# tum-pbs/differentiable-piso

Hardware: AMD Instinct MI355X
Metric: PISO steps/s (fwd+adjoint) at 2048^2 staggered grid (higher is better)
Workload: dtype f64

## Files before the change

### differentiable-piso_amd/csrc/cg.hip

```cpp
#include <atomic>
#include "cg_kernels.h"
#include "cg_driver.h"
#include "cg_tiny.h"
#include "options.h"
#include <cstdio>
#include <vector>

namespace piso {

struct CgProfile {
  int enabled = 0, stride = 8;
  double ms[4] = {0, 0, 0, 0};
  long long count[4] = {0, 0, 0, 0};
};
static CgProfile g_prof;

struct HostPoll {
  CgState* pinned = nullptr;
  hipEvent_t ev[2] = {nullptr, nullptr};
  hipEvent_t seg_ev[2] = {nullptr, nullptr};
  int cus = 0;
};
static std::atomic<unsigned> g_persist_launches{0};
static int g_persist_fallbacks = 0;
static thread_local int tl_xcd_map[kPersistMaxGrid];
static thread_local int tl_xcd_map_n = 0;
static long long g_tiny_solves = 0;
enum { DI_PATH = 0, DI_SIZEOF_T, DI_SIZEOF_CT, DI_V, DI_RECON, DI_SYMMETRIC, DI_ROWS_PER_WAVE, DI_K1_GRID, DI_K1_TILES, DI_R, DI_NQ,
       DI_WAVES, DI_LAUNCH_GRID, DI_PADDED, DI_XCD_LOCAL, DI_FELL_BACK, DI_TINY_PER_X, DI_K2_GRID, DI_SEGMENTS, DI_COUNT };
static thread_local int tl_dispatch[DI_COUNT];
static thread_local int tl_dispatch_n = 0;
static bool g_xcd_local_failed = false;
static long long g_verify_runs = 0;
static int g_verify_failures = 0;
constexpr int kPollDevices = 16;
static thread_local HostPoll tl_poll_dev[kPollDevices];
static thread_local HostPoll* tl_poll_cur = &tl_poll_dev[0];
#define tl_poll (*tl_poll_cur)

static int ensure_poll() {
  int dev = 0;
// ... 180 lines not shown

  int start(unsigned* persist_ws, bool symmetric, int rank_deficient, bool allow_persist) {
    const size_t n = (size_t)a.nx * a.ny;
    tile = cg_tile(a, V, opt(OPT_CG_RPW), opt(OPT_CG_MAXBLOCKS));
    PISO_TRY(ensure_poll());
    if (prof) PISO_TRY(ensure_events(ep));
    ep.used[0] = ep.used[1] = 0;
    prof_stride = g_prof.stride > 0 ? g_prof.stride : 8;
    cg_init<T><<<tile.gflat, kBlock, 0, stream>>>(a, rank_deficient);
    PISO_LAUNCH_CHECK();
    batch = poll_batch(n);
    plan = persist_plan(PersistQuery{a.nx, a.ny, V, a.per_y, a.nx_true != 0, sizeof(T), sizeof(CT), RECON, symmetric, false, tl_poll.cus,
                                     opt(OPT_CG_PERSIST), opt(OPT_CG_PERSIST_R), opt(OPT_CG_PERSIST_HALF), opt(OPT_CG_PERSIST_NQ),
                                     opt(OPT_CG_XCD_LOCAL), g_xcd_local_failed, allow_persist});
    PISO_TRY((persist_prepare<T, CT, RECON, false>(plan, tl_poll.cus, pc, persist_ws, stream)));
    if (plan.R && kPersistDiag && opt_on(OPT_CG_PERSIST_TIMING)) {
      PISO_HIP_CHECK(hipMalloc(reinterpret_cast<void**>(&timing.ticks), 12 * plan.launch_grid * sizeof(unsigned long long)));
      PISO_HIP_CHECK(hipMemsetAsync(timing.ticks, 0, 12 * plan.launch_grid * sizeof(unsigned long long), stream));
      pc.timing = timing.ticks;
    }
    record_dispatch(plan.R ? 3 : 2, sizeof(T), sizeof(CT), 0, V, RECON, symmetric, &tile, &plan, !allow_persist);
    seg_len = persist_segment_len(n, opt(OPT_CG_SEGMENT));
    hipEvent_t* seg_ev = tl_poll.seg_ev;
    if (plan.R && prof && !seg_ev[0]) { PISO_HIP_CHECK(hipEventCreate(&seg_ev[0])); PISO_HIP_CHECK(hipEventCreate(&seg_ev[1])); }
    return PISO_OK;
  }

  bool persistent() const { return plan.R != 0; }
  int segment(int k, int ke, CgLoop& st) {
    hipEvent_t* seg_ev = tl_poll.seg_ev;
// ... 51 lines not shown
    return PISO_OK;
  }
  int look(int k, CgLoop& st) { return (!fixed && (k + 1) % batch == 0 && k + 1 < st.total) ? poll(st, false) : PISO_OK; }

  int finish(CgLoop& st) {
    if (!fixed && !st.finished) PISO_TRY(poll(st, true));
    PISO_HIP_CHECK(hipStreamSynchronize(stream));
    if (opt(OPT_CG_XCD_MAP) == 1) {
      tl_xcd_map_n = 0;
      if (st.segments_run > 0 && !plan.xcd_local && plan.grid <= kPersistMaxGrid) {
        PISO_HIP_CHECK(hipMemcpy(tl_xcd_map, pc.xcd + kPersistXcdTable, (size_t)plan.grid * sizeof(int), hipMemcpyDeviceToHost));
        tl_xcd_map_n = plan.grid;
      }
    }
    if (st.segments_run > 0) {
      int herr = 0;
      PISO_HIP_CHECK(hipMemcpy(&herr, pc.err, sizeof(int), hipMemcpyDeviceToHost));
      if (herr) { ++g_persist_fallbacks; return kPersistRetry; }
    }
    if (st.segments_run > 0 && sizeof(T) == 8 && !fixed && opt(OPT_CG_VERIFY) != 0) {
      bool failed = false;
      PISO_TRY((verify_residual<T, CT>(a, pc, stream, &failed)));
      if (failed) { ++g_verify_failures; ++g_persist_fallbacks; return kPersistRetry; }
    }
    if (timing.ticks) PISO_TRY(print_persist_timing(timing.ticks, plan.grid, st.k_last));
    tl_dispatch[DI_SEGMENTS] = st.segments_run;
    return PISO_OK;
  }
};

template <typename T>
__global__ __launch_bounds__(kBlock) void cg_copy_rows(const T* __restrict__ src, T* __restrict__ dst, int nx, int ny, int ld_src, int ld_dst) {
  const size_t n = (size_t)nx * ny;
// ... 165 lines not shown
                          1 << 30, iterations, nullptr, kernel_ms_out, workspace, workspace_bytes, stream);
}

void piso_cg_profile_enable(int enable, int stride) {
  g_prof.enabled = enable;
  if (stride > 0) g_prof.stride = stride;
  for (int q = 0; q < 4; ++q) { g_prof.ms[q] = 0; g_prof.count[q] = 0; }
}

int piso_cg_persist_fallbacks(void) { return g_persist_fallbacks; }
int piso_cg_last_xcd_map(int* out, int capacity) {
  const int n = tl_xcd_map_n < capacity ? tl_xcd_map_n : capacity;
  for (int i = 0; i < n; ++i) out[i] = tl_xcd_map[i];
  return tl_xcd_map_n;
}
long long piso_cg_tiny_solves(void) { return g_tiny_solves; }
int piso_cg_last_dispatch(int* out, int capacity) {
  const int n = tl_dispatch_n < capacity ? tl_dispatch_n : capacity;
  for (int i = 0; i < n; ++i) out[i] = tl_dispatch[i];
  return tl_dispatch_n;
}
void piso_cg_verify_stats(long long* runs_out, int* failures_out) {
  if (runs_out) *runs_out = g_verify_runs;
  if (failures_out) *failures_out = g_verify_failures;
}

void piso_cg_profile_read(double* ms_sum, long long* count) {
  for (int q = 0; q < 4; ++q) { ms_sum[q] = g_prof.ms[q]; count[q] = g_prof.count[q]; }
}

// ... 2 lines not shown
```

### differentiable-piso_amd/csrc/cg_dispatch.h

```cpp
#pragma once
#include <type_traits>

#include "cg_persist1.h"

namespace piso {

constexpr int kXcdCus = 32;
constexpr int kPersistRetry = -1000;

struct CgTiling { int rows_per_wave, k1_tiles, g1, g2, gflat; };
template <typename T>
inline CgTiling cg_tile(CgArgs<T>& a, int V, int rpw_knob, int maxblocks_knob) {
  const size_t n = (size_t)a.nx * a.ny;
  a.ntx = (a.nx + 64 * V - 1) / (64 * V);
  int rpw = (int)(((long long)a.ny * a.ntx) / (4 * 1024));
  rpw = rpw < 2 ? 2 : (rpw > 16 ? 16 : rpw);
  if (rpw_knob > 0) rpw = rpw_knob;
  a.rows_per_wave = rpw;
  a.nty = (a.ny + 4 * rpw - 1) / (4 * rpw);
  CgTiling t;
  t.rows_per_wave = rpw; t.k1_tiles = a.ntx * a.nty;
  t.g1 = grid_for((long long)t.k1_tiles, 1, (maxblocks_knob >= 8 && maxblocks_knob <= kMaxPartials) ? maxblocks_knob : 1024);
  t.g2 = grid_for((long long)((n / V + kBlock - 1) / kBlock), 4);
  t.gflat = grid_for((long long)n, kBlock * 4);
// ... 117 lines not shown
    one(r, nq, yes, no, no); one(r, nq, yes, yes, no); one(r, nq, yes, no, yes); one(r, nq, yes, yes, yes);
  };
  shape(std::integral_constant<int, 2>{}, std::integral_constant<int, 1>{}); shape(std::integral_constant<int, 2>{}, std::integral_constant<int, 2>{});
  shape(std::integral_constant<int, 4>{}, std::integral_constant<int, 2>{}); shape(std::integral_constant<int, 16>{}, std::integral_constant<int, 1>{});
  return found;
}

template <typename T, typename CT, bool RECON, bool SLAB>
inline int persist_prepare(PersistPlan& p, int cus, PersistCtl& pc, unsigned* ws, hipStream_t stream) {
  int per_cu = 0;
  hipError_t e = hipSuccess;
  const bool have = persist_dispatch<T, CT, RECON, SLAB>(p, [&](auto kfn) { e = hipOccupancyMaxActiveBlocksPerMultiprocessor(&per_cu, kfn, kPersistThreads, 0); });
  if (e != hipSuccess) { set_error("hipOccupancyMaxActiveBlocksPerMultiprocessor", e); return PISO_ERR_HIP; }
  if (!have || (long long)per_cu * cus < p.launch_grid) p.R = 0;
  pc.rec = nullptr; pc.err = nullptr; pc.nreg = p.nreg; pc.ntx = p.ntx; pc.timing = nullptr; pc.epoch0 = 0; pc.xcd = nullptr; pc.local_n = 0; pc.waves = p.waves;
  if (!p.R) return PISO_OK;
  pc.rec = reinterpret_cast<unsigned long long*>(ws);
  pc.err = reinterpret_cast<int*>(ws + kPersistWsWordsAll - 16);
  pc.xcd = reinterpret_cast<int*>(ws + kPersistRecWords);
  pc.local_n = p.xcd_local ? p.grid : 0;
  PISO_HIP_CHECK(hipMemsetAsync(ws, 0, kPersistWsWordsAll * sizeof(unsigned), stream));
  return PISO_OK;
}

template <typename T, typename CT, bool RECON, bool SLAB>
inline int persist_launch(const PersistPlan& p, const CgArgs<T>& a, PersistCtl& pc, unsigned launch_count, int kb, int ke, int sv, bool pending,
                          const std::conditional_t<SLAB, SlabCtl, NoSlab>& sl, hipStream_t stream) {
  pc.epoch0 = (launch_count & 0xffffu) << 16;
  PISO_HIP_CHECK(hipMemsetAsync(pc.rec, 0, kPersistZeroBytes, stream));
  const bool have = persist_dispatch<T, CT, RECON, SLAB>(p, [&](auto kfn) { kfn<<<p.launch_grid, kPersistThreads, 0, stream>>>(a, pc, kb, ke, sv, pending ? 1 : 0, sl); });
// ... 7 lines not shown
```

### differentiable-piso_amd/csrc/cg_persist.h

```cpp
#pragma once
#include "cg_kernels.h"

#define PISO_SB_A1 __builtin_amdgcn_sched_barrier(0)
#define PISO_SB_A2 __builtin_amdgcn_sched_barrier(0)
#define PISO_SB_B1 __builtin_amdgcn_sched_barrier(0)
#define PISO_SB_B2 __builtin_amdgcn_sched_barrier(0)

namespace piso {

constexpr int kPersistThreads = 512;
constexpr int kPersistWaves = kPersistThreads / 64;

struct PersistCtl {
  unsigned long long* rec;
  int* err;
  int nreg, ntx;
  unsigned epoch0;
  unsigned long long* timing;
  int* xcd;
  int local_n;
  int waves;
};
#ifdef PISO_PERSIST_DIAG
constexpr bool kPersistDiag = true;
#else
constexpr bool kPersistDiag = false;
#endif
constexpr int kPersistMaxGrid = 256;
constexpr size_t kPersistRecWords = (size_t)2 * kPersistMaxGrid * 32 + (size_t)2 * 8 * 32;
constexpr int kPersistXcdTable = 16;
constexpr size_t kPersistWsWordsAll = kPersistRecWords + 64 + kPersistMaxGrid;
constexpr size_t kPersistZeroBytes = kPersistRecWords * 4 + 16 * sizeof(int);
// ... 108 lines not shown
```

### differentiable-piso_amd/csrc/cg_persist1.h

```cpp
#pragma once
#include <cstddef>
#include <type_traits>

#include "cg_persist.h"
#include "peer.h"

namespace piso {

struct NoSlab {};
struct SlabCtl {
  PeerView pv;
  double ncells;
  char *rows_own, *rows_lo, *rows_hi;
  unsigned hop_ticks;
};
template <typename T, typename SL>
struct Persist1Kargs { CgArgs<T> a; PersistCtl c; int k_begin, k_end, sv, pend; SL sl; };
template <typename F>
__device__ __forceinline__ F karg(unsigned off) {
  typedef __attribute__((address_space(4))) const char kchar;
  typedef __attribute__((address_space(4))) const unsigned kword;
  kchar* kp = (kchar*)__builtin_amdgcn_kernarg_segment_ptr();
  asm volatile("" : "+s"(kp));
  static_assert(sizeof(F) % 4 == 0, "whole dwords");
// ... 481 lines not shown
  }
}
__device__ __forceinline__ void ring_lane(int lane, int R, int& side, int& er) {
  side = (lane < R) ? 0 : ((lane >= 48 && lane < 48 + R) ? 1 : 2);
  er = (side == 1) ? lane - 48 : lane;
}

constexpr int kSystem = 17;

template <typename T, typename CT, int R, int NQ, bool RECON, bool SYM, bool SLAB = false, bool RAGGED = false, bool LOCAL = false>
__global__ __launch_bounds__(kPersistThreads) void cg_persist1(CgArgs<T> a, PersistCtl c, int k_begin, int k_end, int sv, int pend,
                                                               std::conditional_t<SLAB, SlabCtl, NoSlab> sl = {}) {
  static_assert(!(SLAB && RAGGED), "a slab is never padded");
  static_assert(!(SLAB && LOCAL), "a slab's neighbours are other GPUs");
  constexpr int kPub = LOCAL ? kPlain : kAgent;
  constexpr int kHalo = kAgent;
  constexpr int V = 16 / sizeof(T);
  static_assert(R * NQ <= 16 && 2 * R <= 64, "at most 16 rows per wave; the edge columns of a region fit one wave-wide load");
  static_assert(!SLAB || sizeof(T) == 8, "mailbox rows hold 8-byte elements");
  __shared__ T xs[kPersistWaves * NQ * R * 64 * V];
  __shared__ T smem[2 * kX1Sm + (SLAB ? 2 * kX1SmX : 0)];
  constexpr bool kParkHalos = (NQ * R < 16) || NQ == 1;
  __shared__ T halo_s[kParkHalos ? kPersistWaves * NQ * 2 * 64 * V : 1];
  constexpr bool kRingLds = sizeof(CT) == 4;
  constexpr bool kParkRing = kRingLds;
  constexpr int kRingBytes = 64 * (int)sizeof(T) + 64 * (int)sizeof(CT) + (kParkRing ? 64 * (int)sizeof(T) : 0);
  constexpr unsigned kRingR = 64u * (unsigned)sizeof(T) + 64u * (unsigned)sizeof(CT);
  __shared__ __attribute__((aligned(16))) unsigned char ring_s[kRingLds ? kPersistWaves * NQ * kRingBytes : 16];
  const int nx = a.nx, ny = a.ny;
  const int lane = threadIdx.x & 63;
// ... 84 lines not shown
    zoff = (unsigned)(4 + parity * 2 + side) * cap8;
    return make_rsrc(karg<char*>(sl_off + field_off), on ? 8u * cap8 : 0u);
  };
  const rsrc_t RoS = make_rsrc(a.oS, nbytesC), RoW = make_rsrc(a.oW, nbytesC), RoE = make_rsrc(a.oE, nbytesC), RoN = make_rsrc(a.oN, nbytesC);
  const rsrc_t RcC = make_rsrc(a.cC, nbytesT);
  const rsrc_t Rz0 = make_rsrc(a.zp[0], nbytesT), Rz1 = make_rsrc(a.zp[1], nbytesT);
  auto row_wrap = [&](int j, bool& valid) __attribute__((always_inline)) -> int {
    valid = true;
    if (j < 0) { if (!a.per_y) valid = false; return ny - 1; }
    if (j >= ny) { if (!a.per_y) valid = false; return 0; }
    return j;
  };

  const T alpha0 = pend ? uniform(a.scal[SC_ALPHA]) : (T)0;
  Vec<T, V> rr[NQ][R], pp[NQ][R];
  constexpr bool kPack = R > 2 && V == 2;
  unsigned vT[NQ], vEnd[NQ];
  Vec<T, V> rhb[NQ], rha[NQ], pnb[NQ], pna[NQ];
  T eR[NQ], edge[NQ];
  bool vb[NQ], va[NQ], vl[NQ], vr[NQ];
  unsigned nbits[NQ];
  auto nbit = [&](int q, unsigned bit) __attribute__((always_inline)) -> bool {
    unsigned b = nbits[q];
    asm volatile("" : "+s"(b));
    return (b & bit) != 0;
  };
  {
    const rsrc_t Rr = make_rsrc(a.r, nbytesT), Rx = make_rsrc(a.x, nbytesT), Rp = make_rsrc(a.p[k_begin & 1], nbytesT);
#pragma unroll
    for (int q = 0; q < NQ; ++q) {
      const int cq = (tx0[q] * 64 + lane) * V;
// ... 34 lines not shown
      rha[q] = bld<T, V>(Rr, ha, (unsigned)ja * rowT);
      pnb[q] = bld<T, V>(Rp, hb, (unsigned)jb * rowT);
      pna[q] = bld<T, V>(Rp, ha, (unsigned)ja * rowT);
      if constexpr (kParkHalos) {
        T* hs = halo_s + (size_t)((wave * NQ + q) * 2) * 64 * V + lane * V;
        stv<T, V>(hs, pnb[q]);
        stv<T, V>(hs + 64 * V, pna[q]);
      }
      }
      int side, er;
      ring_lane(lane, R, side, er);
      int cc = (side == 0) ? tx0[q] * 64 * V - 1 : (tx0[q] + 1) * 64 * V;
      vl[q] = tx0[q] > 0 || a.per_x;
      vr[q] = tx0[q] + 1 < c.ntx || a.per_x;
      nbits[q] = (vb[q] ? 1u : 0u) | (va[q] ? 2u : 0u) | (vl[q] ? 4u : 0u) | (vr[q] ? 8u : 0u);
      nbits[q] = (unsigned)__builtin_amdgcn_readfirstlane((int)nbits[q]);
      asm volatile("" : "+s"(nbits[q]));
      if (cc < 0) cc = a.per_x ? nx - 1 : -1;
      else if (cc >= nx) cc = a.per_x ? 0 : -1;
      const unsigned vo = (has[q] && side < 2 && cc >= 0) ? (unsigned)(j0[q] + er) * rowT + (unsigned)(cc * sizeof(T)) : 0xffffffffu;
      eR[q] = bld1<T>(Rr, vo, 0);
      edge[q] = bld1<T>(Rp, vo, 0);
    }
  }
  CgState st = a.state[sv & 1];
  T pz = uniform(a.scal[SC_PZ]), vs = uniform(a.scal[SC_VS]), alpha = uniform(a.scal[SC_ALPHA]);
  const T sc_c = uniform(a.scal[SC_C]);
  T ncells = (T)((double)nx * (double)ny);
  if constexpr (SLAB) ncells = (T)sl.ncells;
  if constexpr (RAGGED) ncells = (T)a.ncells;
// ... 143 lines not shown
    for (int e = 0; e < V; ++e) {
      const T pw = (e == 0) ? left : cur.v[e > 0 ? e - 1 : 0];
      const T pe = (e == V - 1) ? right : cur.v[e < V - 1 ? e + 1 : 0];
      T tmp = 0;
      tmp = fma((T)cS[t].v[e], behind.v[e], tmp);
      tmp = fma((T)cW[t].v[e], pw, tmp);
      tmp = fma(kC.v[e], cur.v[e], tmp);
      tmp = fma((T)kE.v[e], pe, tmp);
      tmp = fma((T)kN.v[e], ahead.v[e], tmp);
      z.v[e] = tmp;
    }
    return z;
  };
  Vec<T, V> zk[kKeepZ ? NT : 1];
  int k = k_begin;
  auto publish = [&](rsrc_t Rd, int q, int jj, const Vec<T, V>& val) __attribute__((always_inline)) {
    const unsigned sT = row_base(q, jj, rowT);
    if (jj == 0 || jj == R - 1) {
      bst<T, V, kPub>(Rd, vT[q], sT, val);
      if constexpr (kPack) bst<T, V, kPub>(Rd, vEnd[q], row_base(q, 1, rowT) + (unsigned)(jj * 16), val);
      if constexpr (SLAB) {
        if (jj == 0) {
          unsigned zoff;
          const rsrc_t Rm = mailbox_rows((unsigned)offsetof(SlabCtl, rows_lo), k & 1, 1, zoff, (ef[q] & 1u) != 0);
          bst<T, V, kSystem>(Rm, vT[q], zoff, val);
        }
        if (jj == R - 1) {
          unsigned zoff;
          const rsrc_t Rm = mailbox_rows((unsigned)offsetof(SlabCtl, rows_hi), k & 1, 0, zoff, (ef[q] & 2u) != 0);
          bst<T, V, kSystem>(Rm, vT[q], zoff, val);
        }
      }
    } else {
      if constexpr (kPack) {
        bst<T, V, kPub>(Rd, vEnd[q], row_base(q, 1, rowT) + (unsigned)(jj * 16), val);
      } else {
        bst<T, V, kPub>(Rd, vEnd[q], sT, val);
      }
    }
  };
  T eZ[NQ];
  Vec<T, V> hbZ[NQ], haZ[NQ];
  auto issue_halos = [&](rsrc_t Rz) __attribute__((always_inline)) {
#pragma unroll
    for (int q = 0; q < NQ; ++q) {
      int side, er, lane_now = lane;
      asm volatile("" : "+v"(lane_now));
      ring_lane(lane_now, R, side, er);
      int cc = (side == 0) ? tx0[q] * 64 * V - 1 : (tx0[q] + 1) * 64 * V;
      if (cc < 0) cc = a.per_x ? nx - 1 : -1;
      else if (cc >= nx) cc = a.per_x ? 0 : -1;
      unsigned vo = (side < 2 && cc >= 0) ? (unsigned)(j0[q] + er) * rowT + (unsigned)(cc * sizeof(T)) : 0xffffffffu;
// ... 41 lines not shown
  unsigned long long tacc[5] = {0, 0, 0, 0, 0}, tsub[4] = {0, 0, 0, 0}, tlast = (kPersistDiag && c.timing) ? wall_clock64() : 0;
  auto tick = [&](int slot) __attribute__((always_inline)) {
    if (kPersistDiag && c.timing) { const unsigned long long t = wall_clock64(); tacc[slot] += t - tlast; tlast = t; }
  };
  if (!st.done && k > 0 && (k % 5) == 0) {
    const int exceeded = tB[2] > 0;
    if (st.flag && !exceeded) { st.done = 1; st.iterations = k; }
    else st.flag = 1;
  }
  T rz_next = tB[0], sumr = tB[1], cnt_last = tB[2];
  T lU[2] = {0, 0};
  const T accuracy = uniform((T)a.accuracy);
  T beta = uniform(-(rz_next + vs * sumr) / pz);
  for (; k < k_end && healthy && !st.done; ++k) {
    rsrc_t Rz;
    if constexpr (SLAB || NT == 16) {
      typedef CgArgs<T> A;
      Rz = make_rsrc(karg<T*>((unsigned)offsetof(KArgs, a) + (unsigned)offsetof(A, zp) + 8u * (unsigned)(k & 1)), nbytesT);
    } else {
      Rz = (k & 1) ? Rz1 : Rz0;
    }
    T sD[kX1Values] = {0, 0, 0, 0, 0, 0, 0, 0};
    if (has[0]) {
#pragma unroll
      for (int q = 0; q < NQ; ++q) {
#pragma unroll
        for (int jj = 0; jj < R; ++jj) {
#pragma unroll
          for (int e = 0; e < V; ++e) pp[q][jj].v[e] = fma(beta, pp[q][jj].v[e], rr[q][jj].v[e]);
        }
        if constexpr (kParkRing) {
          const unsigned rb = ring_a + (unsigned)(q * kRingBytes) + (unsigned)lane * (unsigned)sizeof(T);
          const T e_old = *(lds_T*)(unsigned long)rb, r_col = *(lds_T*)(unsigned long)(rb + kRingR);
          *(lds_T*)(unsigned long)rb = fma(beta, e_old, r_col);
        } else {
// ... 19 lines not shown
#pragma unroll
      for (int t = 0; t < NT; ++t) {
        const int q = t / R, jj = t - q * R;
        if (t + 1 < NT) ring_issue(t + 1);
        const Vec<T, V> z = zrow(t);
        if constexpr (kKeepZ) zk[t] = z;
#pragma unroll
        for (int e = 0; e < V; ++e) {
          sD[0] += pp[q][jj].v[e];
          sD[1] = fma(pp[q][jj].v[e], rr[q][jj].v[e], sD[1]);
          sD[2] = fma(pp[q][jj].v[e], z.v[e], sD[2]);
          sD[3] = fma(rr[q][jj].v[e], z.v[e], sD[3]);
          sD[4] = fma(z.v[e], z.v[e], sD[4]);
          sD[5] += z.v[e];
        }
        publish(Rz, q, jj, z);
        PISO_SB_A1;
        if constexpr (D < NT) { if (t + D < NT) issue_coef(t + D); }
        if constexpr (kShLate) { if (t + D == NT - 1) reload_csh(); }
        PISO_SB_A2;
      }
    }
    sD[6] = lU[0]; sD[7] = lU[1];
    ++epoch;
    tick(0);
    Vec<T, V> zs[kAhead > 0 ? kAhead : 1];
    auto z_ahead = [&]() __attribute__((always_inline)) {
      if constexpr (kAhead > 0) {
        if (has[0]) {
          ring_issue(NT - 1);
#pragma unroll
// ... 16 lines not shown
        if (st.flag && !exceeded) { st.done = 1; st.iterations = k; }
        else st.flag = 1;
      }
      if (st.done) break;
    }
    first = false;
    vs = uniform(sc_c * sD[0]);
    pz = uniform(sD[2] + vs * sD[0]);
    alpha = uniform((absval(pz) > 0) ? sD[1] / pz : (T)0);
    rz_next = uniform(sD[3] - alpha * (sD[4] + vs * sD[5]));
    sumr = uniform(sumr - alpha * (sD[5] + ncells * vs));
    beta = uniform(-(rz_next + vs * sumr) / pz);
    lU[0] = 0; lU[1] = 0;
    int cnt_wave = 0;
    if (has[0]) {
      issue_halos(Rz);
      if constexpr (kAhead < NT && !kKeepZ) ring_issue(NT - 1 - kAhead);
#pragma unroll
      for (int tt = 0; tt < NT; ++tt) {
        const int t = NT - 1 - tt;
        const int q = t / R, jj = t - q * R;
        if constexpr (!kKeepZ) { if (tt + 1 < NT && tt + 1 > kAhead) ring_issue(t - 1); }
        T* xl = xs + (size_t)(wave * NQ + q) * R * 64 * V + lane * V + jj * 64 * V;
        Vec<T, V> xv = ldv<T, V>(xl);
        Vec<T, V> z;
        if constexpr (kKeepZ) z = zk[t];
        else z = (tt < kAhead) ? zs[tt < kAhead ? tt : 0] : zrow(t);
#pragma unroll
        for (int e = 0; e < V; ++e) xv.v[e] = fma(alpha, pp[q][jj].v[e], xv.v[e]);
        stv<T, V>(xl, xv);
// ... 134 lines not shown
```

### differentiable-piso_amd/csrc/cg_slab.hip

```cpp
#include <vector>

#include "cg_driver.h"
#include "cg_kernels.h"
#include "options.h"
#include "peer.h"
#include "slab_comm.h"

namespace piso {

struct SlabRank {
  CgArgs<double> a;
  double *rbase, *pbase[2], *xbase;
  double* g;
  double* oT; float* oF; double* cC;
  int* flags;
  const double* L;
  double* x_out;
  int rank;
  unsigned* persist_ws;
};

template <typename T>
__global__ __launch_bounds__(kBlock) void slab_collapse(const T* __restrict__ parts, int records, int count, T* __restrict__ out) {
  __shared__ T smem[16];
// ... 101 lines not shown
      const CgTiling tile = cg_tile(a, V, 0, 0);
      g1[q] = tile.g1; g2[q] = tile.g2; gflat[q] = tile.gflat;
      a.accuracy = accuracy;
      a.gA = R[q].g; a.gB = R[q].g + 4;
    }
    if (!tl_slab_pinned) PISO_HIP_CHECK(hipHostMalloc(reinterpret_cast<void**>(&tl_slab_pinned), sizeof(SlabPinned), hipHostMallocDefault));
    int cus = 0;
    if (allow_persist && comm.peer() && nloc == 1 && R[0].a.nx <= (int)comm.rccl->row_cap) {
      int dev = 0;
      PISO_HIP_CHECK(hipGetDevice(&dev));
      PISO_HIP_CHECK(hipDeviceGetAttribute(&cus, hipDeviceAttributeMultiprocessorCount, dev));
      plan = persist_plan(PersistQuery{R[0].a.nx, R[0].a.ny, V, R[0].a.per_y, false, sizeof(double), sizeof(CT), RECON, symmetric, true, cus,
                                       opt(OPT_CG_PERSIST), opt(OPT_CG_PERSIST_R), 0, 0, 0, false, true});
    }
    PISO_TRY((persist_prepare<double, CT, RECON, true>(plan, cus, pc, R[0].persist_ws, stream)));
    if (plan.R) {
      sl.pv = make_view(comm.rccl, comm.periodic_y);
      sl.ncells = global_cells;
      sl.rows_own = sl.pv.mbox[sl.pv.rank] + PeerLayout::kRows;
      sl.rows_lo = sl.pv.mbox[sl.pv.lower >= 0 ? sl.pv.lower : sl.pv.rank] + PeerLayout::kRows;
      sl.rows_hi = sl.pv.mbox[sl.pv.upper >= 0 ? sl.pv.upper : sl.pv.rank] + PeerLayout::kRows;
      sl.hop_ticks = opt(OPT_SLAB_HOP_TICKS) > 0 ? (unsigned)opt(OPT_SLAB_HOP_TICKS) : 0u;
    }
    seg_len = persist_segment_len((size_t)R[0].a.nx * R[0].a.ny, opt(OPT_CG_SEGMENT));
    return PISO_OK;
  }

  bool persistent() const { return plan.R != 0; }
  int segment(int k, int ke, CgLoop& st) {
    PisoComm* c = comm.rccl;
// ... 210 lines not shown
```

### differentiable-piso_amd/csrc/options.h

```cpp
#pragma once

namespace piso {

enum Opt {
  OPT_CG_PERSIST = 0,
  OPT_CG_PERSIST_R,
  OPT_CG_PERSIST_HALF,
  OPT_CG_PERSIST_NQ,
  OPT_CG_SEGMENT,
  OPT_CG_PERSIST_TIMING,
  OPT_CG_RPW,
  OPT_CG_MAXBLOCKS,
  OPT_CG_NT,
  OPT_CG_NO_COMPACT,
  OPT_CG_NO_RECON,
  OPT_CG_NO_SYM,
  OPT_CG_VERIFY,
  OPT_CG_PAD,
  OPT_CG_XCD_LOCAL,
  OPT_CG_TINY,
  OPT_CG_XCD_MAP,
  OPT_CONV_LDS,
  OPT_BICG_FOLD,
  OPT_BICG_SWEEP_LDS,
  OPT_BICG_FUSE_P,
  OPT_SLAB_FORCE,
  OPT_SLAB_HOP_TICKS,
  OPT_MG_TAIL,
  OPT_MG_CHECK_EVERY,
  OPT_COUNT
};

int opt(Opt o);
inline bool opt_on(Opt o) { return opt(o) > 0; }

struct OptScope {
// ... 8 lines not shown
```

### differentiable-piso_amd/csrc/runtime.hip

```cpp
#include "piso_common.h"
#include "options.h"
#include <stdlib.h>
#include <atomic>

namespace piso {
static thread_local char g_err[512] = "";
void set_error(const char* what, hipError_t err) {
  snprintf(g_err, sizeof(g_err), "%s: %s", what, hipGetErrorString(err));
}
void set_error_msg(const char* what) { snprintf(g_err, sizeof(g_err), "%s", what); }

static const char* const kOptNames[OPT_COUNT] = {"cg_persist", "cg_persist_r", "cg_persist_half", "cg_persist_nq", "cg_segment", "cg_persist_timing",
                                                 "cg_rpw", "cg_maxblocks", "cg_nt", "cg_no_compact", "cg_no_recon", "cg_no_sym", "cg_verify", "cg_pad", "cg_xcd_local", "cg_tiny", "cg_xcd_map", "conv_lds", "bicg_fold", "bicg_sweep_lds", "bicg_fuse_p", "slab_force", "slab_hop_ticks", "mg_tail", "mg_check_every"};
struct Options {
  std::atomic<int> v[OPT_COUNT];
  Options() {
    for (int i = 0; i < OPT_COUNT; ++i) {
      char env[64] = "PISO_";
      size_t k = 5;
      for (const char* c = kOptNames[i]; *c && k + 1 < sizeof(env); ++c) env[k++] = (char)((*c >= 'a' && *c <= 'z') ? *c - 32 : *c);
      env[k] = 0;
      const char* e = getenv(env);
      v[i].store((e && *e) ? atoi(e) : -1, std::memory_order_relaxed);
    }
    if (getenv("PISO_CG_NO_PERSIST")) v[OPT_CG_PERSIST].store(0, std::memory_order_relaxed);
  }
};
static Options g_opt;
// ... 38 lines not shown
```

### differentiable-piso_amd/diffpiso/_native.py

```python
import ctypes as C
import os

import torch

_HERE = os.path.dirname(os.path.abspath(__file__))
LIB_PATH = os.environ.get("PISO_HIP_LIB") or os.path.join(_HERE, "libpiso_hip.so")

if not os.path.isfile(LIB_PATH):
    raise ImportError('HIP binaries not found at %s. Run "python differentiable-piso_amd/build_native.py" '
                      '(or __graft_entry__.build()) to compile them' % LIB_PATH)

lib = C.CDLL(LIB_PATH)

_vp, _i, _f, _sz = C.c_void_p, C.c_int, C.c_float, C.c_size_t
_ip = C.POINTER(C.c_int)

lib.piso_version.restype = C.c_char_p
lib.piso_last_error_string.restype = C.c_char_p
lib.piso_device_count.restype = _i
lib.piso_set_option.argtypes = [C.c_char_p, _i]
lib.piso_set_option.restype = _i
lib.piso_get_option.argtypes = [C.c_char_p, _ip]
lib.piso_get_option.restype = _i
lib.piso_cg_persist_fallbacks.restype = _i
lib.piso_cg_last_xcd_map.argtypes = [_ip, _i]
lib.piso_cg_last_xcd_map.restype = _i
lib.piso_cg_tiny_solves.restype = C.c_longlong
lib.piso_cg_last_dispatch.argtypes = [_ip, _i]
lib.piso_cg_last_dispatch.restype = _i
lib.piso_bicgstab_last_dispatch.argtypes = [_ip, _i]
lib.piso_bicgstab_last_dispatch.restype = _i
lib.piso_conv_last_dispatch.argtypes = [_ip, _i]
lib.piso_conv_last_dispatch.restype = _i
lib.piso_cg_verify_stats.argtypes = [C.POINTER(C.c_longlong), _ip]
lib.piso_cg_verify_stats.restype = None
lib.piso_csr_nnz.argtypes = [_i, _i, _i, _i, _ip, _ip]
lib.piso_csr_nnz.restype = None
lib.piso_assemble_csr.argtypes = [_vp, _vp, _vp, _vp, _vp, _vp, _vp, _vp, _i, _i, _i, _i, _i, _f, _f, _f, _f, _vp, _f, _vp]
lib.piso_assemble_csr.restype = _i
for _n in ("piso_laplace_matrix_f64", "piso_laplace_matrix_f32"):
    getattr(lib, _n).argtypes = [_i, _i, _vp, _vp, _vp, _vp, _vp]
# ... 219 lines not shown
```

### include/piso_hip.h

```cpp
#ifndef PISO_HIP_H
#define PISO_HIP_H

#include <stddef.h>
#include <stdint.h>

#ifdef __cplusplus
extern "C" {
#endif

#define PISO_OK 0
#define PISO_ERR_INVALID_ARG 1
#define PISO_ERR_HIP 2
#define PISO_ERR_UNSUPPORTED_PATTERN 3
#define PISO_ERR_NO_DEVICE 4
#define PISO_ERR_NEEDS_HOST 5

typedef void* piso_stream_t;

typedef struct piso_slab {
  int ny_global;
  int row_begin, row_end;
  int owns_last_face_row;
} piso_slab_t;

// ... 89 lines not shown
int piso_cg_solve_async_f64(int nx, int ny, int periodic_x, int periodic_y, const double* laplace, const double* divergence,
                            double* x_out, float accuracy, int max_iterations, int rank_deficient, int residual_reset,
                            int* iterations_dev, void* workspace, size_t workspace_bytes, piso_stream_t stream);
int piso_cg_solve_async_f32(int nx, int ny, int periodic_x, int periodic_y, const float* laplace, const float* divergence,
                            float* x_out, float accuracy, int max_iterations, int rank_deficient, int residual_reset,
                            int* iterations_dev, void* workspace, size_t workspace_bytes, piso_stream_t stream);

int piso_cg_fixed_iterations_f64(int nx, int ny, int periodic_x, int periodic_y, const double* laplace,
                                 const double* divergence, double* x_out, int rank_deficient, int iterations,
                                 float* kernel_ms_out, void* workspace, size_t workspace_bytes, piso_stream_t stream);

void piso_cg_profile_enable(int enable, int stride);
void piso_cg_profile_read(double* ms_sum, long long* count);
int piso_cg_persist_fallbacks(void);
int piso_cg_last_xcd_map(int* out, int capacity);
long long piso_cg_tiny_solves(void);
int piso_cg_last_dispatch(int* out, int capacity);
void piso_cg_verify_stats(long long* runs_out, int* failures_out);

size_t piso_mg_workspace_bytes(int nx, int ny);
int piso_mg_pcg_solve_f64(int nx, int ny, int periodic_x, int periodic_y, const double* laplace, const double* divergence,
                          double* x_out, float accuracy, int max_iterations, int rank_deficient, int residual_reset,
                          int sweeps, int* iterations_out, void* workspace, size_t workspace_bytes, piso_stream_t stream);
int piso_mg_vcycle_f64(int nx, int ny, int periodic_x, int periodic_y, const double* laplace, const double* r_in, double* z_out,
                       int sweeps, void* workspace, size_t workspace_bytes, piso_stream_t stream);
int piso_mg_level_f64(int nx, int ny, int periodic_x, int periodic_y, const double* laplace, int level, int* nx_out, int* ny_out,
                      double* laplace_level_out, void* workspace, size_t workspace_bytes, piso_stream_t stream);
int piso_mg_last_dispatch(int* out, int capacity);

size_t piso_conv2d_weight_elems(int ks, int cin, int cout);
// ... 51 lines not shown
```

Baseline: 5.194.

## Publish halo rows with plain stores when all neighbour readers share the XCD

```diff
diff --git a/differentiable-piso_amd/csrc/cg.hip b/differentiable-piso_amd/csrc/cg.hip
--- a/differentiable-piso_amd/csrc/cg.hip
+++ b/differentiable-piso_amd/csrc/cg.hip
@@ -25,6 +25,7 @@
 static int g_persist_fallbacks = 0;
 static thread_local int tl_xcd_map[kPersistMaxGrid];
 static thread_local int tl_xcd_map_n = 0;
+static thread_local int tl_pub_plain = 0, tl_pub_total = 0;
 static long long g_tiny_solves = 0;
 enum { DI_PATH = 0, DI_SIZEOF_T, DI_SIZEOF_CT, DI_V, DI_RECON, DI_SYMMETRIC, DI_ROWS_PER_WAVE, DI_K1_GRID, DI_K1_TILES, DI_R, DI_NQ,
        DI_WAVES, DI_LAUNCH_GRID, DI_PADDED, DI_XCD_LOCAL, DI_FELL_BACK, DI_TINY_PER_X, DI_K2_GRID, DI_SEGMENTS, DI_COUNT };
@@ -235,6 +236,8 @@
                                      opt(OPT_CG_PERSIST), opt(OPT_CG_PERSIST_R), opt(OPT_CG_PERSIST_HALF), opt(OPT_CG_PERSIST_NQ),
                                      opt(OPT_CG_XCD_LOCAL), g_xcd_local_failed, allow_persist});
     PISO_TRY((persist_prepare<T, CT, RECON, false>(plan, tl_poll.cus, pc, persist_ws, stream)));
+    pc.pub_scope = opt(OPT_CG_PUB_SCOPE) != 0 ? 1 : 0;
+    tl_pub_plain = tl_pub_total = 0;
     if (plan.R && kPersistDiag && opt_on(OPT_CG_PERSIST_TIMING)) {
       PISO_HIP_CHECK(hipMalloc(reinterpret_cast<void**>(&timing.ticks), 12 * plan.launch_grid * sizeof(unsigned long long)));
       PISO_HIP_CHECK(hipMemsetAsync(timing.ticks, 0, 12 * plan.launch_grid * sizeof(unsigned long long), stream));
@@ -316,9 +319,16 @@
       }
     }
     if (st.segments_run > 0) {
-      int herr = 0;
-      PISO_HIP_CHECK(hipMemcpy(&herr, pc.err, sizeof(int), hipMemcpyDeviceToHost));
+      constexpr int kTail = (int)(kPersistWsWordsAll - 16 - kPersistRecWords) - kPersistXcdTable + 1;
+      static thread_local int tail[kTail];
+      PISO_HIP_CHECK(hipMemcpy(tail, pc.xcd + kPersistXcdTable, sizeof(tail), hipMemcpyDeviceToHost));
+      const int herr = tail[kTail - 1];
       if (herr) { ++g_persist_fallbacks; return kPersistRetry; }
+      if (!plan.xcd_local && pub_scope_instance(RECON, plan.sym)) {
+        const PubShape shape = {plan.launch_grid, plan.waves, plan.NQ, plan.nreg, plan.ntx, a.per_x ? 1 : 0, a.per_y ? 1 : 0, pub_pack(plan.R, V) ? 1 : 0};
+        pub_count_sides(shape, tail, &tl_pub_plain, &tl_pub_total);
+        if (!pc.pub_scope) tl_pub_plain = 0;
+      }
     }
     if (st.segments_run > 0 && sizeof(T) == 8 && !fixed && opt(OPT_CG_VERIFY) != 0) {
       bool failed = false;
@@ -514,6 +524,20 @@
   for (int i = 0; i < n; ++i) out[i] = tl_xcd_map[i];
   return tl_xcd_map_n;
 }
+void piso_cg_pub_plain_sides(int* plain, int* total) {
+  if (plain) *plain = tl_pub_plain;
+  if (total) *total = tl_pub_total;
+}
+int piso_cg_pub_scope_predicate(const int* table, int grid, int waves, int nq, int nreg, int ntx, int wrap_x, int wrap_y, int pack, unsigned* bits_out) {
+  if (!table || !bits_out || grid < 1 || grid > kPersistMaxGrid || waves < 1 || nq < 1 || ntx < 1 || nreg < 1 || nreg % ntx != 0 ||
+      (nreg + waves * nq - 1) / (waves * nq) != grid) {
+    set_error_msg("piso_cg_pub_scope_predicate: not the shape of a chip-wide persistent launch");
+    return PISO_ERR_INVALID_ARG;
+  }
+  const PubShape shape = {grid, waves, nq, nreg, ntx, wrap_x ? 1 : 0, wrap_y ? 1 : 0, pack ? 1 : 0};
+  for (int reg = 0; reg < nreg; ++reg) bits_out[reg] = pub_plain_sides(shape, reg, [&](int b) { return table[b]; });
+  return PISO_OK;
+}
 long long piso_cg_tiny_solves(void) { return g_tiny_solves; }
 int piso_cg_last_dispatch(int* out, int capacity) {
   const int n = tl_dispatch_n < capacity ? tl_dispatch_n : capacity;
diff --git a/differentiable-piso_amd/csrc/cg_dispatch.h b/differentiable-piso_amd/csrc/cg_dispatch.h
--- a/differentiable-piso_amd/csrc/cg_dispatch.h
+++ b/differentiable-piso_amd/csrc/cg_dispatch.h
@@ -155,6 +155,7 @@
   if (e != hipSuccess) { set_error("hipOccupancyMaxActiveBlocksPerMultiprocessor", e); return PISO_ERR_HIP; }
   if (!have || (long long)per_cu * cus < p.launch_grid) p.R = 0;
   pc.rec = nullptr; pc.err = nullptr; pc.nreg = p.nreg; pc.ntx = p.ntx; pc.timing = nullptr; pc.epoch0 = 0; pc.xcd = nullptr; pc.local_n = 0; pc.waves = p.waves;
+  pc.pub_scope = 0;
   if (!p.R) return PISO_OK;
   pc.rec = reinterpret_cast<unsigned long long*>(ws);
   pc.err = reinterpret_cast<int*>(ws + kPersistWsWordsAll - 16);
diff --git a/differentiable-piso_amd/csrc/cg_persist.h b/differentiable-piso_amd/csrc/cg_persist.h
--- a/differentiable-piso_amd/csrc/cg_persist.h
+++ b/differentiable-piso_amd/csrc/cg_persist.h
@@ -16,6 +16,7 @@
   int* err;
   int nreg, ntx;
   unsigned epoch0;
+  int pub_scope;
   unsigned long long* timing;
   int* xcd;
   int local_n;
diff --git a/differentiable-piso_amd/csrc/cg_persist1.h b/differentiable-piso_amd/csrc/cg_persist1.h
--- a/differentiable-piso_amd/csrc/cg_persist1.h
+++ b/differentiable-piso_amd/csrc/cg_persist1.h
@@ -3,6 +3,7 @@
 #include <type_traits>
 
 #include "cg_persist.h"
+#include "cg_pub_scope.h"
 #include "peer.h"
 
 namespace piso {
@@ -519,6 +520,7 @@
   static_assert(!(SLAB && RAGGED), "a slab is never padded");
   static_assert(!(SLAB && LOCAL), "a slab's neighbours are other GPUs");
   constexpr int kPub = LOCAL ? kPlain : kAgent;
+  constexpr bool kPubScope = !LOCAL && pub_scope_instance(RECON, SYM);
   constexpr int kHalo = kAgent;
   constexpr int V = 16 / sizeof(T);
   static_assert(R * NQ <= 16 && 2 * R <= 64, "at most 16 rows per wave; the edge columns of a region fit one wave-wide load");
@@ -633,7 +635,7 @@
 
   const T alpha0 = pend ? uniform(a.scal[SC_ALPHA]) : (T)0;
   Vec<T, V> rr[NQ][R], pp[NQ][R];
-  constexpr bool kPack = R > 2 && V == 2;
+  constexpr bool kPack = pub_pack(R, V);
   unsigned vT[NQ], vEnd[NQ];
   Vec<T, V> rhb[NQ], rha[NQ], pnb[NQ], pna[NQ];
   T eR[NQ], edge[NQ];
@@ -698,6 +700,14 @@
       vl[q] = tx0[q] > 0 || a.per_x;
       vr[q] = tx0[q] + 1 < c.ntx || a.per_x;
       nbits[q] = (vb[q] ? 1u : 0u) | (va[q] ? 2u : 0u) | (vl[q] ? 4u : 0u) | (vr[q] ? 8u : 0u);
+      if constexpr (kHier) {
+        if (kPubScope && c.pub_scope && has[q]) {
+          const int* const table = c.xcd + kPersistXcdTable;
+          const PubShape shape = {(int)gridDim.x, c.waves, NQ, c.nreg, c.ntx, a.per_x ? 1 : 0, (!SLAB && a.per_y) ? 1 : 0, kPack ? 1 : 0};
+          nbits[q] |= pub_plain_sides(shape, (j0[q] / R) * c.ntx + tx0[q],
+                                      [&](int b) { return __hip_atomic_load(table + b, __ATOMIC_RELAXED, __HIP_MEMORY_SCOPE_AGENT); });
+        }
+      }
       nbits[q] = (unsigned)__builtin_amdgcn_readfirstlane((int)nbits[q]);
       asm volatile("" : "+s"(nbits[q]));
       if (cc < 0) cc = a.per_x ? nx - 1 : -1;
@@ -871,11 +881,20 @@
   };
   Vec<T, V> zk[kKeepZ ? NT : 1];
   int k = k_begin;
-  auto publish = [&](rsrc_t Rd, int q, int jj, const Vec<T, V>& val) __attribute__((always_inline)) {
+  auto pub_store = [&](int q, unsigned side, rsrc_t Rd, const T* zb, unsigned voff, unsigned soff, const Vec<T, V>& val) __attribute__((always_inline)) {
+    if constexpr (kPubScope) {
+      const bool plain = nbit(q, side);
+      bst<T, V, kPlain>(make_rsrc(zb, (unsigned)__builtin_amdgcn_readfirstlane((int)(plain ? nbytesT : 0u))), voff, soff, val);
+      bst<T, V, kAgent>(make_rsrc(zb, (unsigned)__builtin_amdgcn_readfirstlane((int)(plain ? 0u : nbytesT))), voff, soff, val);
+    } else {
+      bst<T, V, kPub>(Rd, voff, soff, val);
+    }
+  };
+  auto publish = [&](rsrc_t Rd, const T* zb, int q, int jj, const Vec<T, V>& val) __attribute__((always_inline)) {
     const unsigned sT = row_base(q, jj, rowT);
     if (jj == 0 || jj == R - 1) {
-      bst<T, V, kPub>(Rd, vT[q], sT, val);
-      if constexpr (kPack) bst<T, V, kPub>(Rd, vEnd[q], row_base(q, 1, rowT) + (unsigned)(jj * 16), val);
+      pub_store(q, jj == 0 ? kPubRowLo : kPubRowHi, Rd, zb, vT[q], sT, val);
+      if constexpr (kPack) pub_store(q, kPubEnds, Rd, zb, vEnd[q], row_base(q, 1, rowT) + (unsigned)(jj * 16), val);
       if constexpr (SLAB) {
         if (jj == 0) {
           unsigned zoff;
@@ -890,9 +909,9 @@
       }
     } else {
       if constexpr (kPack) {
-        bst<T, V, kPub>(Rd, vEnd[q], row_base(q, 1, rowT) + (unsigned)(jj * 16), val);
+        pub_store(q, kPubEnds, Rd, zb, vEnd[q], row_base(q, 1, rowT) + (unsigned)(jj * 16), val);
       } else {
-        bst<T, V, kPub>(Rd, vEnd[q], sT, val);
+        pub_store(q, kPubEnds, Rd, zb, vEnd[q], sT, val);
       }
     }
   };
@@ -964,11 +983,14 @@
   T beta = uniform(-(rz_next + vs * sumr) / pz);
   for (; k < k_end && healthy && !st.done; ++k) {
     rsrc_t Rz;
+    const T* zb;
     if constexpr (SLAB || NT == 16) {
       typedef CgArgs<T> A;
-      Rz = make_rsrc(karg<T*>((unsigned)offsetof(KArgs, a) + (unsigned)offsetof(A, zp) + 8u * (unsigned)(k & 1)), nbytesT);
+      zb = karg<T*>((unsigned)offsetof(KArgs, a) + (unsigned)offsetof(A, zp) + 8u * (unsigned)(k & 1));
+      if constexpr (!(SLAB && kPubScope)) Rz = make_rsrc(zb, nbytesT);
     } else {
       Rz = (k & 1) ? Rz1 : Rz0;
+      zb = a.zp[k & 1];
     }
     T sD[kX1Values] = {0, 0, 0, 0, 0, 0, 0, 0};
     if (has[0]) {
@@ -1018,7 +1040,7 @@
           sD[4] = fma(z.v[e], z.v[e], sD[4]);
           sD[5] += z.v[e];
         }
-        publish(Rz, q, jj, z);
+        publish(Rz, zb, q, jj, z);
         PISO_SB_A1;
         if constexpr (D < NT) { if (t + D < NT) issue_coef(t + D); }
         if constexpr (kShLate) { if (t + D == NT - 1) reload_csh(); }
@@ -1065,6 +1087,10 @@
     lU[0] = 0; lU[1] = 0;
     int cnt_wave = 0;
     if (has[0]) {
+      if constexpr (SLAB && kPubScope) {
+        typedef CgArgs<T> A;
+        Rz = make_rsrc(karg<T*>((unsigned)offsetof(KArgs, a) + (unsigned)offsetof(A, zp) + 8u * (unsigned)(k & 1)), nbytesT);
+      }
       issue_halos(Rz);
       if constexpr (kAhead < NT && !kKeepZ) ring_issue(NT - 1 - kAhead);
 #pragma unroll
diff --git a/differentiable-piso_amd/csrc/cg_pub_scope.h b/differentiable-piso_amd/csrc/cg_pub_scope.h
--- /dev/null
+++ b/differentiable-piso_amd/csrc/cg_pub_scope.h
@@ -0,0 +1,69 @@
+#pragma once
+
+#if defined(__HIPCC__)
+#define PISO_PUB_HD __host__ __device__
+#else
+#define PISO_PUB_HD
+#endif
+
+namespace piso {
+
+constexpr unsigned kPubRowLo = 16u;
+constexpr unsigned kPubRowHi = 32u;
+constexpr unsigned kPubEnds = 64u;
+constexpr unsigned kPubAll = kPubRowLo | kPubRowHi | kPubEnds;
+constexpr int kPubXcds = 8;
+
+struct PubShape {
+  int grid;
+  int waves, nq;
+  int nreg, ntx;
+  int wrap_x, wrap_y;
+  int pack;
+};
+
+PISO_PUB_HD constexpr bool pub_pack(int R, int V) { return R > 2 && V == 2; }
+
+PISO_PUB_HD constexpr bool pub_scope_instance(bool recon, bool sym) { return recon || sym; }
+
+PISO_PUB_HD inline int pub_wg_of_block(int b, int grid) {
+  return (grid % kPubXcds == 0) ? (b % kPubXcds) * (grid / kPubXcds) + b / kPubXcds : b;
+}
+PISO_PUB_HD inline int pub_block_of_wg(int wg, int grid) {
+  return (grid % kPubXcds == 0) ? (wg % (grid / kPubXcds)) * kPubXcds + wg / (grid / kPubXcds) : wg;
+}
+PISO_PUB_HD inline int pub_block_of_region(const PubShape& s, int reg) { return pub_block_of_wg(reg / (s.waves * s.nq), s.grid); }
+
+struct PubReaders { int below, above, left, right; };
+PISO_PUB_HD inline PubReaders pub_readers(const PubShape& s, int reg) {
+  const int nty = s.nreg / s.ntx, ty = reg / s.ntx, tx = reg - ty * s.ntx;
+  PubReaders r;
+  r.below = ty > 0 ? reg - s.ntx : (s.wrap_y ? (nty - 1) * s.ntx + tx : -1);
+  r.above = ty + 1 < nty ? reg + s.ntx : (s.wrap_y ? tx : -1);
+  r.left = tx > 0 ? reg - 1 : (s.wrap_x ? reg + s.ntx - 1 : -1);
+  r.right = tx + 1 < s.ntx ? reg + 1 : (s.wrap_x ? reg - (s.ntx - 1) : -1);
+  return r;
+}
+
+template <typename XcdOfBlock>
+PISO_PUB_HD inline unsigned pub_plain_sides(const PubShape& s, int reg, XcdOfBlock&& xcd_of_block) {
+  const int mine = xcd_of_block(pub_block_of_region(s, reg));
+  const PubReaders r = pub_readers(s, reg);
+  const bool below = r.below < 0 || xcd_of_block(pub_block_of_region(s, r.below)) == mine;
+  const bool above = r.above < 0 || xcd_of_block(pub_block_of_region(s, r.above)) == mine;
+  const bool ends = (r.left < 0 || xcd_of_block(pub_block_of_region(s, r.left)) == mine) &&
+                    (r.right < 0 || xcd_of_block(pub_block_of_region(s, r.right)) == mine);
+  const bool rows_hold_ends = !s.pack;
+  return ((below && (ends || !rows_hold_ends)) ? kPubRowLo : 0u) | ((above && (ends || !rows_hold_ends)) ? kPubRowHi : 0u) | (ends ? kPubEnds : 0u);
+}
+
+inline void pub_count_sides(const PubShape& s, const int* table, int* plain, int* total) {
+  int n = 0;
+  for (int reg = 0; reg < s.nreg; ++reg) {
+    const unsigned bits = pub_plain_sides(s, reg, [&](int b) { return table[b]; });
+    n += ((bits & kPubRowLo) ? 1 : 0) + ((bits & kPubRowHi) ? 1 : 0) + ((bits & kPubEnds) ? 1 : 0);
+  }
+  *plain = n; *total = 3 * s.nreg;
+}
+
+}
diff --git a/differentiable-piso_amd/csrc/cg_slab.hip b/differentiable-piso_amd/csrc/cg_slab.hip
--- a/differentiable-piso_amd/csrc/cg_slab.hip
+++ b/differentiable-piso_amd/csrc/cg_slab.hip
@@ -139,6 +139,7 @@
                                        opt(OPT_CG_PERSIST), opt(OPT_CG_PERSIST_R), 0, 0, 0, false, true});
     }
     PISO_TRY((persist_prepare<double, CT, RECON, true>(plan, cus, pc, R[0].persist_ws, stream)));
+    pc.pub_scope = opt(OPT_CG_PUB_SCOPE) != 0 ? 1 : 0;
     if (plan.R) {
       sl.pv = make_view(comm.rccl, comm.periodic_y);
       sl.ncells = global_cells;
diff --git a/differentiable-piso_amd/csrc/options.h b/differentiable-piso_amd/csrc/options.h
--- a/differentiable-piso_amd/csrc/options.h
+++ b/differentiable-piso_amd/csrc/options.h
@@ -20,6 +20,7 @@
   OPT_CG_XCD_LOCAL,
   OPT_CG_TINY,
   OPT_CG_XCD_MAP,
+  OPT_CG_PUB_SCOPE,
   OPT_CONV_LDS,
   OPT_BICG_FOLD,
   OPT_BICG_SWEEP_LDS,
diff --git a/differentiable-piso_amd/csrc/runtime.hip b/differentiable-piso_amd/csrc/runtime.hip
--- a/differentiable-piso_amd/csrc/runtime.hip
+++ b/differentiable-piso_amd/csrc/runtime.hip
@@ -11,7 +11,7 @@
 void set_error_msg(const char* what) { snprintf(g_err, sizeof(g_err), "%s", what); }
 
 static const char* const kOptNames[OPT_COUNT] = {"cg_persist", "cg_persist_r", "cg_persist_half", "cg_persist_nq", "cg_segment", "cg_persist_timing",
-                                                 "cg_rpw", "cg_maxblocks", "cg_nt", "cg_no_compact", "cg_no_recon", "cg_no_sym", "cg_verify", "cg_pad", "cg_xcd_local", "cg_tiny", "cg_xcd_map", "conv_lds", "bicg_fold", "bicg_sweep_lds", "bicg_fuse_p", "slab_force", "slab_hop_ticks", "mg_tail", "mg_check_every"};
+                                                 "cg_rpw", "cg_maxblocks", "cg_nt", "cg_no_compact", "cg_no_recon", "cg_no_sym", "cg_verify", "cg_pad", "cg_xcd_local", "cg_tiny", "cg_xcd_map", "cg_pub_scope", "conv_lds", "bicg_fold", "bicg_sweep_lds", "bicg_fuse_p", "slab_force", "slab_hop_ticks", "mg_tail", "mg_check_every"};
 struct Options {
   std::atomic<int> v[OPT_COUNT];
   Options() {
diff --git a/differentiable-piso_amd/diffpiso/_native.py b/differentiable-piso_amd/diffpiso/_native.py
--- a/differentiable-piso_amd/diffpiso/_native.py
+++ b/differentiable-piso_amd/diffpiso/_native.py
@@ -25,6 +25,10 @@
 lib.piso_cg_persist_fallbacks.restype = _i
 lib.piso_cg_last_xcd_map.argtypes = [_ip, _i]
 lib.piso_cg_last_xcd_map.restype = _i
+lib.piso_cg_pub_plain_sides.argtypes = [_ip, _ip]
+lib.piso_cg_pub_plain_sides.restype = None
+lib.piso_cg_pub_scope_predicate.argtypes = [_ip, _i, _i, _i, _i, _i, _i, _i, _i, C.POINTER(C.c_uint)]
+lib.piso_cg_pub_scope_predicate.restype = _i
 lib.piso_cg_tiny_solves.restype = C.c_longlong
 lib.piso_cg_last_dispatch.argtypes = [_ip, _i]
 lib.piso_cg_last_dispatch.restype = _i
diff --git a/include/piso_hip.h b/include/piso_hip.h
--- a/include/piso_hip.h
+++ b/include/piso_hip.h
@@ -127,6 +127,9 @@
 void piso_cg_profile_read(double* ms_sum, long long* count);
 int piso_cg_persist_fallbacks(void);
 int piso_cg_last_xcd_map(int* out, int capacity);
+void piso_cg_pub_plain_sides(int* plain, int* total);
+int piso_cg_pub_scope_predicate(const int* table, int grid, int waves, int nq, int nreg, int ntx, int wrap_x, int wrap_y, int pack,
+                                unsigned* bits_out);
 long long piso_cg_tiny_solves(void);
 int piso_cg_last_dispatch(int* out, int capacity);
 void piso_cg_verify_stats(long long* runs_out, int* failures_out);
```

New measurement: 4.886. 5.9% lower.
